# hzdr/PARIS

Hardware: AMD Instinct MI355X
Metric: GVoxel-updates/s (voxels x projections / s), FDK hot path weight+filter+backproject (higher is better)
Workload: dtype f32

## Files before the change

paris_amd/csrc/backproject.hip:

```cpp
#include "bp_device.h"

#include <mutex>
#include <utility>

namespace
{
    __global__ void __launch_bounds__(256) fastdiv_validate_kernel(float c, float r, unsigned long long* mismatches)
    {
        const uint32_t t = blockIdx.x * 256u + threadIdx.x;
        unsigned int bad = 0;
        for(uint32_t i = 0; i < 256u; ++i)
        {
            const uint32_t bits = (i << 24) | t;
            const float x = __uint_as_float(bits);
            const float want = x / c - (1.f / 2.f);
            const float got = div_by_constant(x, c, r) - (1.f / 2.f);
            const bool same = __float_as_uint(want) == __float_as_uint(got);
            const bool both_nan = (want != want) && (got != got);
            const bool want_far = !(fabsf(want) <= 16777216.f);
            const bool got_far = !(fabsf(got) <= 16777216.f);
            if(!(same || both_nan || (want_far && got_far)))
                ++bad;
        }
        if(bad)
// ... 256 lines not shown
}

int paris_hip_prevalidate_fast_division(paris_hip_ctx* ctx, float l_px_row, float l_px_col)
{
    if(ctx == nullptr || ctx->bp_fastdiv == 0)
        return PARIS_HIP_SUCCESS;
    bool ok = false;
    if(int rc = fastdiv_is_exact(ctx, l_px_row, &ok))
        return rc;
    return fastdiv_is_exact(ctx, l_px_col, &ok);
}

int paris_hip_prevalidate_lean_division(paris_hip_ctx* ctx, float d_so, float d_od)
{
    if(ctx == nullptr || ctx->bp_lean_div == 0)
        return PARIS_HIP_SUCCESS;
    bool ok = false;
    return paris_hip_lean_division_check(ctx, std::fabs(d_so) + std::fabs(d_od), d_so, &ok);
}

static int volume_stream_policy(const paris_hip_ctx* ctx, uint32_t v_dim_x, uint32_t v_dim_y, uint32_t v_dim_z)
{
    if(ctx->bp_nt >= 0)
        return ctx->bp_nt;
    const uint64_t bytes = 4ull * v_dim_x * v_dim_y * v_dim_z;
    return bytes <= (384ull << 20) ? 0 : 2;
}

static int fill_params(paris_hip_ctx* ctx, const void* d_p, bool f16, size_t p_pitch, uint32_t p_dim_x, uint32_t p_dim_y,
                       float* d_v, uint32_t v_dim_x, uint32_t v_dim_y, uint32_t v_dim_z, uint32_t v_offset,
                       const paris_detector_geometry* det_geo, const paris_volume_geometry* vol_geo, int enable_roi,
                       const paris_region_of_interest* roi, float sin_phi, float cos_phi, float delta_s, float delta_t,
                       BpParams& g, bool& fd, bool& skip)
{
    const size_t px = f16 ? sizeof(uint16_t) : sizeof(float);
    skip = false;
    if(int rc = paris_hip_bind(ctx))
        return rc;
    if(int rc = paris_hip_flush_pending_weight(ctx))
        return rc;
    if(d_p == nullptr || d_v == nullptr || det_geo == nullptr || vol_geo == nullptr || (enable_roi && roi == nullptr))
        return PARIS_HIP_ERROR_INVALID_ARGUMENT;
    if(p_dim_x == 0 || p_dim_y == 0 || p_pitch < static_cast<size_t>(p_dim_x) * px || p_pitch % px != 0)
        return PARIS_HIP_ERROR_INVALID_ARGUMENT;
    if(v_dim_x == 0 || v_dim_y == 0 || v_dim_z == 0)
    {
        skip = true;
        return PARIS_HIP_SUCCESS;
    }
    const uint64_t plane = static_cast<uint64_t>(v_dim_x) * v_dim_y;
    const uint32_t tz_auto = plane > (1ull << 20) ? (v_dim_z <= 256u ? 8u : TZ_DEFAULT) : (plane > (1ull << 18) ? 8u : TZ_DEFAULT);
    const uint32_t tz = ctx->bp_tz ? ctx->bp_tz : tz_auto;
    {
        const uint32_t tz_min = std::min(tz, 8u);
        const uint64_t ntx = (v_dim_x + 63u) / 64u, nty = (v_dim_y + 3u) / 4u, ntz = (v_dim_z + tz_min - 1u) / tz_min;
        const uint64_t zchunk = chunk_tiles(12u, tz_min, static_cast<uint32_t>(ntz), 64u);
        const uint64_t padded = std::max<uint64_t>(8ull * (8u * ((nty + 63u) / 64u)) * ntx * zchunk * ((ntz + zchunk - 1u) / zchunk),
                                                   8ull * ntx * nty * (ntz / 8u) + 8ull * 7u * 8u * ((nty + 63u) / 64u) * ntx);
        if(padded > 0x7fffff00ull)
            return PARIS_HIP_ERROR_UNSUPPORTED;
    }

    g = BpParams{};
    g.proj = d_p;
    g.proj_f16 = f16 ? 1u : 0u;
    g.vol = d_v;
    g.p_pitch = static_cast<uint32_t>(p_pitch / px);
    g.p_dim_x = p_dim_x;
    g.p_dim_y = p_dim_y;
    g.v_dim_x = v_dim_x;
    g.v_dim_y = v_dim_y;
    g.v_dim_z = v_dim_z;
    g.k_off = enable_roi ? roi->x1 : 0u;
    g.l_off = enable_roi ? roi->y1 : 0u;
    g.m_off = (enable_roi ? roi->z1 : 0u) + v_offset;
    g.x_base = centered_base(vol_geo->dim_x, vol_geo->l_vx_x);
    g.y_base = centered_base(vol_geo->dim_y, vol_geo->l_vx_y);
    g.z_base = centered_base(vol_geo->dim_z, vol_geo->l_vx_z);
    g.l_vx_x = vol_geo->l_vx_x;
    g.l_vx_y = vol_geo->l_vx_y;
    g.l_vx_z = vol_geo->l_vx_z;
    g.sin_phi = sin_phi;
    g.cos_phi = cos_phi;
    g.d_so = det_geo->d_so;
    g.d_sd = std::fabs(det_geo->d_so) + std::fabs(det_geo->d_od);
    g.l_px_x = det_geo->l_px_row;
    g.l_px_y = det_geo->l_px_col;
    g.min_h = detector_min(p_dim_x, g.l_px_x, delta_s);
    g.min_v = detector_min(p_dim_y, g.l_px_y, delta_t);
    g.rcp_l_px_y = 1.f / g.l_px_y;
    g.rcp_l_px_x = 1.f / g.l_px_x;
    fd = false;
    if(ctx->bp_fastdiv != 0)
    {
        bool fd_x = false;
        if(int rc = fastdiv_is_exact(ctx, g.l_px_y, &fd))
            return rc;
        if(int rc = fastdiv_is_exact(ctx, g.l_px_x, &fd_x))
            return rc;
        fd = fd && fd_x;
    }
    {
        const double x0 = g.x_base + static_cast<double>(g.k_off) * g.l_vx_x, x1 = g.x_base + (static_cast<double>(g.k_off) + v_dim_x - 1.0) * g.l_vx_x;
        const double y0 = g.y_base + static_cast<double>(g.l_off) * g.l_vx_y, y1 = g.y_base + (static_cast<double>(g.l_off) + v_dim_y - 1.0) * g.l_vx_y;
        const double reach = std::hypot(std::max(std::fabs(x0), std::fabs(x1)), std::max(std::fabs(y0), std::fabs(y1)));
        const double lo = std::ldexp(1.0, -40), hi = std::ldexp(1.0, 40);
        const bool ordinary = g.d_so >= lo && g.d_so <= hi && g.d_sd >= lo && g.d_sd <= hi;
        g.lean_div = (ctx->bp_lean_div != 0 && ordinary && std::isfinite(reach) && reach <= 0.9 * g.d_so) ? 1u : 0u;
        if(g.lean_div != 0u)
        {
            bool exact = false;
            if(int rc = paris_hip_lean_division_check(ctx, g.d_sd, g.d_so, &exact))
// ... 10 lines not shown
    {
#ifdef PARIS_HIP_EXPERIMENTS
        static const int tile_nest = std::getenv("PARIS_TILE_NEST") ? std::atoi(std::getenv("PARIS_TILE_NEST")) : -1;
#else
        constexpr int tile_nest = -1;
#endif
        g.yfast = tile_nest >= 0 ? static_cast<uint32_t>(tile_nest) : (v_dim_z > 256u ? 2u : 0u);
    }
    g.order = ctx->bp_order >= 0 ? static_cast<uint32_t>(ctx->bp_order) : (plane > (1ull << 20) ? 15u : 18u);
    g.store_sc1 = volume_stream_policy(ctx, v_dim_x, v_dim_y, v_dim_z) == 2 ? 1u : 0u;
    g.stage_vec4 = (ctx->bp_stage_vec4 != 0 && g.p_pitch % 4u == 0 && reinterpret_cast<uintptr_t>(d_p) % (4u * px) == 0)
                       ? 1u : 0u;
    return PARIS_HIP_SUCCESS;
}

static int lane_width(const float* d_v, uint32_t v_dim_x)
{
    const uintptr_t addr = reinterpret_cast<uintptr_t>(d_v);
    if(v_dim_x % 4u == 0 && addr % 16u == 0)
        return 4;
    if(v_dim_x % 2u == 0 && addr % 8u == 0)
        return 2;
    return 1;
}

static int backproject_impl(paris_hip_ctx* ctx, const void* d_p, bool f16, size_t p_pitch, uint32_t p_dim_x,
                            uint32_t p_dim_y, float* d_v, uint32_t v_dim_x, uint32_t v_dim_y, uint32_t v_dim_z,
                            uint32_t v_offset, const paris_detector_geometry* det_geo,
                            const paris_volume_geometry* vol_geo, int enable_roi, const paris_region_of_interest* roi,
                            float sin_phi, float cos_phi, float delta_s, float delta_t)
{
    BpParams g;
    bool fd = false, skip = false;
    if(int rc = fill_params(ctx, d_p, f16, p_pitch, p_dim_x, p_dim_y, d_v, v_dim_x, v_dim_y, v_dim_z, v_offset, det_geo, vol_geo,
                            enable_roi, roi, sin_phi, cos_phi, delta_s, delta_t, g, fd, skip))
        return rc;
    if(skip)
        return paris_hip_finish(ctx);

    const bool timed = !ctx->bp_start.empty();
    const size_t ev = timed ? static_cast<size_t>(ctx->bp_launches % ctx->bp_start.size()) : 0u;
    if(timed)
        PARIS_HIP_TRY(hipEventRecord(ctx->bp_start[ev], ctx->stream));
    if(ctx->bp_variant == 4 && !f16)
    {
        FusedParams fp{};
        fp.g = g;
        fp.n_proj = 1;
        fp.proj_tab[0] = d_p;
        fp.sin_phi[0] = sin_phi;
        fp.cos_phi[0] = cos_phi;
        const int width = lane_width(d_v, v_dim_x);
        const int vx = ctx->bp_vx == 4 && width == 4 ? 4 : (ctx->bp_vx == 1 || width < 2 ? 1 : 2);
        paris_hip_bp_launch_fused(&fp, vx, ctx->bp_tz == 8u ? 8 : (ctx->bp_tz == 32u ? 32 : 16), volume_stream_policy(ctx, v_dim_x, v_dim_y, v_dim_z) != 0, fd, ctx->stream);
    }
    else
    if(ctx->bp_variant == 1)
    {
        const dim3 grid((v_dim_x + 255u) / 256u, v_dim_y, v_dim_z);
        if(v_dim_y > 65535u || v_dim_z > 65535u)
            return PARIS_HIP_ERROR_UNSUPPORTED;
        hipLaunchKernelGGL(bp_gather_kernel, grid, dim3(256), 0, ctx->stream, g);
    }
    else
    {
        int vx = lane_width(d_v, v_dim_x);
        if(ctx->bp_vx && ctx->bp_vx < vx)
            vx = ctx->bp_vx;
        if(ctx->bp_vx == 0 && vx == 4 && ctx->bp_variant != 3 && ctx->bp_variant != 5)
        {
            const uint64_t tiles = static_cast<uint64_t>((v_dim_x + 63u) / 64u) * ((v_dim_y + 15u) / 16u) * ((v_dim_z + g.tz - 1u) / g.tz);
            if(tiles < 2048u)
                vx = 2;
        }
        const bool deep_big = g.tz == 16u && ctx->bp_tz == 0u && static_cast<uint64_t>(v_dim_x) * v_dim_y > (1ull << 20);
        if(deep_big && ctx->bp_unroll == 0 && ctx->bp_lds_bytes == 0u && vx == 4)
            g.lds_floats = 40u * 1024u / sizeof(float);
        const int unroll = ctx->bp_unroll ? ctx->bp_unroll : ((g.tz == 8u && ctx->bp_tz == 0u) || (deep_big && ctx->bp_lds_bytes == 0u && vx == 4) ? 1 : 2);
        const bool nt = volume_stream_policy(ctx, v_dim_x, v_dim_y, v_dim_z) != 0;
#ifdef PARIS_HIP_EXPERIMENTS
        const bool want_slice = ctx->bp_variant == 3;
        if(want_slice && vx == 4)
        {
            const int nw = ctx->bp_slice_nw ? ctx->bp_slice_nw : 16;
            const int rpl = ctx->bp_slice_rpl ? ctx->bp_slice_rpl : 4;
            const uint32_t box_bytes = ctx->bp_lds_bytes ? ctx->bp_lds_bytes : LDS_BYTES_DEFAULT;
            if(int rc = launch_slice_shape(g, nw, rpl, box_bytes, nt, fd, ctx->stream))
                return rc;
        }
        else if(vx == 4 && ctx->bp_variant == 5 && v_dim_y <= 65535u)
        {
            const size_t need = 3u * static_cast<size_t>(v_dim_x) * v_dim_y;
            if(ctx->colstate_floats < need)
            {
                if(ctx->colstate != nullptr)
                {
                    PARIS_HIP_TRY(hipStreamSynchronize(ctx->stream));
                    PARIS_HIP_TRY(hipFree(ctx->colstate));
                    ctx->colstate = nullptr;
                }
                PARIS_HIP_TRY(hipMalloc(reinterpret_cast<void**>(&ctx->colstate), need * sizeof(float)));
                ctx->colstate_floats = need;
            }
            g.colstate = ctx->colstate;
            if(unroll == 1)
                fd ? launch_tile_pre<1, true>(g, ctx->stream) : launch_tile_pre<1, false>(g, ctx->stream);
            else
// ... 491 lines not shown
    hipLaunchKernelGGL(to_half_kernel, grid, dim3(256), 0, ctx->stream, d_src, static_cast<uint32_t>(src_pitch / sizeof(float)),
                       reinterpret_cast<_Float16*>(d_dst), static_cast<uint32_t>(dst_pitch / sizeof(uint16_t)), dim_x, dim_y);
    if(int rc = paris_hip_note_projection_use(ctx, d_src, src_pitch * dim_y))
        return rc;
    if(int rc = paris_hip_note_projection_use(ctx, d_dst, dst_pitch * dim_y))
        return rc;
    return paris_hip_finish(ctx);
}

extern "C" int paris_hip_backproject_batch(paris_hip_ctx* ctx, const float* d_p, size_t p_pitch,
                                           size_t p_stride_bytes, uint32_t n_proj, uint32_t p_dim_x,
                                           uint32_t p_dim_y, float* d_v, uint32_t v_dim_x, uint32_t v_dim_y,
                                           uint32_t v_dim_z, uint32_t v_offset,
                                           const paris_detector_geometry* det_geo,
                                           const paris_volume_geometry* vol_geo, int enable_roi,
                                           const paris_region_of_interest* roi, const float* sin_phi,
                                           const float* cos_phi, float delta_s, float delta_t)
{
    if(int rc = paris_hip_flush_deferred(ctx))
        return rc;
    return batch_impl(ctx, d_p, false, p_pitch, p_stride_bytes, n_proj, p_dim_x, p_dim_y, d_v, v_dim_x, v_dim_y, v_dim_z, v_offset, det_geo,
                      vol_geo, enable_roi, roi, sin_phi, cos_phi, delta_s, delta_t);
}

extern "C" int paris_hip_backproject_batch_f16(paris_hip_ctx* ctx, const uint16_t* d_p, size_t p_pitch, size_t p_stride_bytes,
                                               uint32_t n_proj, uint32_t p_dim_x, uint32_t p_dim_y, float* d_v, uint32_t v_dim_x,
                                               uint32_t v_dim_y, uint32_t v_dim_z, uint32_t v_offset,
                                               const paris_detector_geometry* det_geo, const paris_volume_geometry* vol_geo,
                                               int enable_roi, const paris_region_of_interest* roi, const float* sin_phi,
                                               const float* cos_phi, float delta_s, float delta_t)
{
    if(int rc = paris_hip_flush_deferred(ctx))
        return rc;
    return batch_impl(ctx, d_p, true, p_pitch, p_stride_bytes, n_proj, p_dim_x, p_dim_y, d_v, v_dim_x, v_dim_y, v_dim_z, v_offset, det_geo,
                      vol_geo, enable_roi, roi, sin_phi, cos_phi, delta_s, delta_t);
}

static int batch_impl(paris_hip_ctx* ctx, const void* d_p, bool f16, size_t p_pitch, size_t p_stride_bytes, uint32_t n_proj, uint32_t p_dim_x,
                      uint32_t p_dim_y, float* d_v, uint32_t v_dim_x, uint32_t v_dim_y, uint32_t v_dim_z, uint32_t v_offset,
                      const paris_detector_geometry* det_geo, const paris_volume_geometry* vol_geo, int enable_roi,
                      const paris_region_of_interest* roi, const float* sin_phi, const float* cos_phi, float delta_s, float delta_t,
                      const void* const* ptrs)
{
    const size_t px = f16 ? sizeof(uint16_t) : sizeof(float);
    if(ctx == nullptr || sin_phi == nullptr || cos_phi == nullptr || (ptrs == nullptr && p_stride_bytes % px != 0))
        return PARIS_HIP_ERROR_INVALID_ARGUMENT;
    if(n_proj == 0)
        return paris_hip_finish(ctx);
    if(ptrs == nullptr && n_proj > 1 && p_stride_bytes < p_pitch * static_cast<size_t>(p_dim_y))
        return PARIS_HIP_ERROR_INVALID_ARGUMENT;
    const auto where = [&](uint32_t i) { return ptrs != nullptr ? static_cast<const char*>(ptrs[i]) : static_cast<const char*>(d_p) + static_cast<size_t>(i) * p_stride_bytes; };

    const int width = d_v != nullptr ? lane_width(d_v, v_dim_x) : 1;
    bool deep_box_fits = true;
    {
        const double d_so = std::fabs(static_cast<double>(det_geo->d_so)), d_sd = d_so + std::fabs(static_cast<double>(det_geo->d_od));
        const double mag = d_so > 0.0 ? d_sd / d_so : 1.0;
        const double rows = 32.0 * vol_geo->l_vx_z * mag / det_geo->l_px_col + 4.0 * std::max(vol_geo->l_vx_x, vol_geo->l_vx_y) * mag / det_geo->l_px_col + 8.0;
        const double cols = 64.0 * std::max(vol_geo->l_vx_x, vol_geo->l_vx_y) * mag / det_geo->l_px_row + 16.0;
        const double budget = ctx->bp_lds_bytes != 0u ? ctx->bp_lds_bytes : 32.0 * 1024.0;
        deep_box_fits = std::isfinite(rows) && std::isfinite(cols) && rows * std::max(132.0, cols) * sizeof(float) <= budget;
    }
    int fused_vx = ((v_dim_z <= 16u || !deep_box_fits) && width >= 2) ? 2 : 1;
    if(ctx->bp_vx == 4 && width == 4)
        fused_vx = 4;
    else if(ctx->bp_vx == 2 && width >= 2)
        fused_vx = 2;
    else if(ctx->bp_vx == 1)
        fused_vx = 1;
    int fused_tz = fused_vx == 1 ? ((v_dim_z <= 16u || !deep_box_fits) ? 16 : 32) : 16;
    if(ctx->bp_tz == 8u && fused_vx != 1)
        fused_tz = 8;
    else if(ctx->bp_tz == 16u)
        fused_tz = 16;
    else if(ctx->bp_tz == 32u && fused_vx == 1)
        fused_tz = 32;
    const bool fused_ok = n_proj > 1 && (ctx->bp_variant == 0 || ctx->bp_variant == 4) && d_v != nullptr;
    if(!fused_ok)
    {
        const unsigned saved = ctx->flags;
        ctx->flags &= ~PARIS_HIP_CTX_SYNCHRONOUS;
        int rc = PARIS_HIP_SUCCESS;
        for(uint32_t i = 0; i < n_proj && rc == PARIS_HIP_SUCCESS; ++i)
        {
            const char* p = where(i);
            rc = backproject_impl(ctx, p, f16, p_pitch, p_dim_x, p_dim_y, d_v, v_dim_x, v_dim_y, v_dim_z, v_offset, det_geo, vol_geo,
                                  enable_roi, roi, sin_phi[i], cos_phi[i], delta_s, delta_t);
        }
        ctx->flags = saved;
        if(rc != PARIS_HIP_SUCCESS)
            return rc;
        return paris_hip_finish(ctx);
    }

    const bool nt = volume_stream_policy(ctx, v_dim_x, v_dim_y, v_dim_z) != 0;
    for(uint32_t first = 0; first < n_proj; first += FUSED_MAX)
    {
        const uint32_t n = std::min<uint32_t>(FUSED_MAX, n_proj - first);
        FusedParams fp{};
        bool fd = false, skip = false;
        const char* p0 = where(first);
        if(int rc = fill_params(ctx, p0, f16, p_pitch, p_dim_x, p_dim_y, d_v, v_dim_x, v_dim_y, v_dim_z, v_offset, det_geo,
                                vol_geo, enable_roi, roi, sin_phi[first], cos_phi[first], delta_s, delta_t, fp.g, fd, skip))
            return rc;
        if(skip)
            break;
        fp.n_proj = n;
        if(ctx->bp_order < 0 && fp.g.order == 15u)
            fp.g.order = fused_vx == 1 ? 17u : (fused_vx == 2 ? 16u : 15u);
#ifdef PARIS_HIP_EXPERIMENTS
        static const bool x_fast = std::getenv("PARIS_FUSED_XFAST") != nullptr;
#else
        constexpr bool x_fast = false;
#endif
        fp.g.yfast = x_fast ? 0u : 1u;
        if(ctx->bp_lds_bytes == 0u)
            fp.g.lds_floats = 32u * 1024u / sizeof(float);
        for(uint32_t i = 0; i < n; ++i)
        {
            fp.sin_phi[i] = sin_phi[first + i];
            fp.cos_phi[i] = cos_phi[first + i];
            fp.proj_tab[i] = where(first + i);
            if(reinterpret_cast<uintptr_t>(fp.proj_tab[i]) % (4u * px) != 0)
                fp.g.stage_vec4 = 0u;
        }
        for(uint32_t i = n; i < FUSED_MAX; ++i)
            fp.proj_tab[i] = fp.proj_tab[0];
        const bool timed = !ctx->bp_start.empty();
        const size_t ev = timed ? static_cast<size_t>(ctx->bp_launches % ctx->bp_start.size()) : 0u;
        if(timed)
            PARIS_HIP_TRY(hipEventRecord(ctx->bp_start[ev], ctx->stream));
        paris_hip_bp_launch_fused(&fp, fused_vx, fused_tz, nt, fd, ctx->stream);
        if(timed)
            PARIS_HIP_TRY(hipEventRecord(ctx->bp_stop[ev], ctx->stream));
        ++ctx->bp_launches;
        for(uint32_t i = 0; i < n && !ctx->upload_targets.empty(); ++i)
            if(int rc = paris_hip_note_projection_use(ctx, where(first + i), p_pitch * p_dim_y))
                return rc;
    }
    return paris_hip_finish(ctx);
}

extern "C" int paris_hip_last_backproject_ms(paris_hip_ctx* ctx, float* ms)
{
    if(int rc = paris_hip_flush_deferred(ctx))
        return rc;
    if(ctx == nullptr || ms == nullptr || ctx->bp_launches == 0 || ctx->bp_start.empty())
        return PARIS_HIP_ERROR_INVALID_ARGUMENT;
    if(int rc = paris_hip_bind(ctx))
        return rc;
    const size_t ev = static_cast<size_t>((ctx->bp_launches - 1) % ctx->bp_start.size());
    PARIS_HIP_TRY(hipEventSynchronize(ctx->bp_stop[ev]));
    PARIS_HIP_TRY(hipEventElapsedTime(ms, ctx->bp_start[ev], ctx->bp_stop[ev]));
    return PARIS_HIP_SUCCESS;
}

extern "C" int paris_hip_set_backproject_variant(paris_hip_ctx* ctx, int variant)
{
    if(int rc = paris_hip_flush_deferred(ctx))
        return rc;
    if(ctx == nullptr || variant < 0 || variant > 5)
        return PARIS_HIP_ERROR_INVALID_ARGUMENT;
#ifndef PARIS_HIP_EXPERIMENTS
    if(variant == 3 || variant == 5)
        return PARIS_HIP_ERROR_UNSUPPORTED;
#endif
    ctx->bp_variant = variant;
    return PARIS_HIP_SUCCESS;
}

extern "C" int paris_hip_set_backproject_order(paris_hip_ctx* ctx, int order, int nontemporal)
{
    if(int rc = paris_hip_flush_deferred(ctx))
        return rc;
    if(ctx == nullptr || !(order == -1 || order == 0 || order == 1 || order == 5 || order == 8 || order == 9 || order == 12 || (order >= 14 && order <= 18)) || nontemporal < -1 || nontemporal > 2)
        return PARIS_HIP_ERROR_INVALID_ARGUMENT;
#ifndef PARIS_HIP_EXPERIMENTS
    if(order == 0 || order == 1 || order == 8 || order == 9 || order == 12)
        return PARIS_HIP_ERROR_UNSUPPORTED;
#endif
    ctx->bp_order = order;
    ctx->bp_nt = nontemporal;
    return PARIS_HIP_SUCCESS;
}

// ... 1 lines not shown
{
    if(int rc = paris_hip_bind(ctx))
        return rc;
    if(exact == nullptr)
        return PARIS_HIP_ERROR_INVALID_ARGUMENT;
    bool ok = false;
    const int saved = ctx->async_validate;
    ctx->async_validate = 0;
    const int rc = fastdiv_is_exact(ctx, divisor, &ok);
    ctx->async_validate = saved;
    if(rc != PARIS_HIP_SUCCESS)
        return rc;
    *exact = ok ? 1 : 0;
    return PARIS_HIP_SUCCESS;
}

extern "C" int paris_hip_set_backproject_vector_staging(paris_hip_ctx* ctx, int enable)
{
    if(int rc = paris_hip_flush_deferred(ctx))
        return rc;
    if(ctx == nullptr)
        return PARIS_HIP_ERROR_INVALID_ARGUMENT;
    ctx->bp_stage_vec4 = enable ? 1 : 0;
    return PARIS_HIP_SUCCESS;
}

extern "C" int paris_hip_set_backproject_skip_invalid(paris_hip_ctx* ctx, int enable)
{
    if(int rc = paris_hip_flush_deferred(ctx))
        return rc;
    if(ctx == nullptr)
        return PARIS_HIP_ERROR_INVALID_ARGUMENT;
    ctx->bp_skip_invalid = enable ? 1 : 0;
    return PARIS_HIP_SUCCESS;
}

extern "C" int paris_hip_set_backproject_fast_division(paris_hip_ctx* ctx, int enable)
{
    if(int rc = paris_hip_flush_deferred(ctx))
        return rc;
    if(ctx == nullptr)
        return PARIS_HIP_ERROR_INVALID_ARGUMENT;
    ctx->bp_lean_div = enable ? 1 : 0;
    ctx->bp_fastdiv = enable ? 1 : 0;
    return PARIS_HIP_SUCCESS;
}

extern "C" int paris_hip_set_backproject_slice_shape(paris_hip_ctx* ctx, int waves, int row_groups)
{
    if(int rc = paris_hip_flush_deferred(ctx))
        return rc;
    if(ctx == nullptr)
        return PARIS_HIP_ERROR_INVALID_ARGUMENT;
    const bool ok = (waves == 0 && row_groups == 0) || (waves == 16 && (row_groups == 4 || row_groups == 2))
                    || (waves == 8 && (row_groups == 4 || row_groups == 2 || row_groups == 1));
    if(!ok)
        return PARIS_HIP_ERROR_INVALID_ARGUMENT;
#ifndef PARIS_HIP_EXPERIMENTS
    if(waves != 0)
        return PARIS_HIP_ERROR_UNSUPPORTED;
#endif
    ctx->bp_slice_nw = waves;
    ctx->bp_slice_rpl = row_groups;
    return PARIS_HIP_SUCCESS;
}

extern "C" int paris_hip_set_backproject_tuning(paris_hip_ctx* ctx, int vx, int unroll, int tz, int lds_bytes)
{
    if(int rc = paris_hip_flush_deferred(ctx))
        return rc;
    if(ctx == nullptr)
        return PARIS_HIP_ERROR_INVALID_ARGUMENT;
    if(!(vx == 0 || vx == 1 || vx == 2 || vx == 4) || !(unroll == 0 || unroll == 1 || unroll == 2 || unroll == 3 || unroll == 4))
        return PARIS_HIP_ERROR_INVALID_ARGUMENT;
    if(tz < 0 || tz > 4096 || lds_bytes < 0 || lds_bytes > static_cast<int>(LDS_BYTES_MAX)
       || (lds_bytes != 0 && lds_bytes < 1024))
        return PARIS_HIP_ERROR_INVALID_ARGUMENT;
#ifndef PARIS_HIP_EXPERIMENTS
    if(unroll > 2)
        return PARIS_HIP_ERROR_UNSUPPORTED;
#endif
    ctx->bp_vx = vx;
    ctx->bp_unroll = unroll;
    ctx->bp_tz = static_cast<uint32_t>(tz);
    ctx->bp_lds_bytes = static_cast<uint32_t>(lds_bytes);
    return PARIS_HIP_SUCCESS;
}

extern "C" int paris_hip_has_experiments(void)
{
#ifdef PARIS_HIP_EXPERIMENTS
    return 1;
#else
    return 0;
#endif
}
```

paris_amd/csrc/backproject_fused.hip:

```cpp
#define PARIS_BP_SINGLE_INSTRUCTION_FLOOR 1
#if (defined(PARIS_TIMING_ONLY_NO_BARRIERS) || defined(PARIS_TIMING_ONLY_STAGE_ONCE)) && !defined(PARIS_HIP_EXPERIMENTS)
#error "the timing-only switches compute WRONG results: they exist in the experiments build only (make EXPERIMENTS=1)"
#endif
#include "bp_device.h"

namespace
{
#ifndef PARIS_FUSED_PIPELINE
#define PARIS_FUSED_PIPELINE 1
#endif
#ifndef PARIS_FUSED_WAVES
#define PARIS_FUSED_WAVES 3
#endif
    constexpr int FIXED_STRIDE = 132;

    template <int VX, int TZ, bool NT, bool FD>
    __global__ void __launch_bounds__(256, PARIS_FUSED_WAVES + (VX == 2 ? 1 : VX == 1 ? (TZ == 32 ? 1 : 4) : 0) + (TZ == 8 ? 1 : 0)) bp_fused_kernel(const FusedParams fp)
    {
        extern __shared__ __attribute__((aligned(16))) float lds[];
        BpParams g = fp.g;
        using vec = typename vec_of<VX>::type;
        constexpr uint32_t XL = 64u / VX;
        constexpr uint32_t RW = VX;
        constexpr uint32_t TY = 4u * RW;

        const uint32_t tid = threadIdx.x;
        const uint32_t lane = tid & 63u;
        const uint32_t wave = tid >> 6;

        uint32_t bx, by, bz;
        if(!tile_of_block(g, blockIdx.x, bx, by, bz))
            return;
        const uint32_t k0 = bx * 64u;
        const uint32_t l0 = by * TY;
        const uint32_t m0 = bz * TZ;
        const uint32_t k1 = min(k0 + 63u, g.v_dim_x - 1u);
        const uint32_t l1 = min(l0 + TY - 1u, g.v_dim_y - 1u);
        const uint32_t m1 = min(m0 + TZ - 1u, g.v_dim_z - 1u);
        const uint32_t mcount = m1 - m0 + 1u;

        const uint32_t xq = lane % XL, yy = lane / XL;
        const uint32_t k = k0 + xq * VX;
        const uint32_t l = l0 + wave * RW + yy;
        const bool active = k < g.v_dim_x && l < g.v_dim_y;

        const size_t slice = static_cast<size_t>(g.v_dim_x) * g.v_dim_y;
        float* vp = g.vol + (static_cast<size_t>(m0) * g.v_dim_y + l) * g.v_dim_x + k;
        vec acc[TZ] = {};
#pragma unroll
        for(int z = 0; z < TZ; ++z)
            if(active && static_cast<uint32_t>(z) < mcount)
                acc[z] = load_voxels<VX, NT>(vp + z * slice);

        const float z_first = g.z_base + static_cast<float>(g.m_off + m0) * g.l_vx_z;
        const float z_last = g.z_base + static_cast<float>(g.m_off + m1) * g.l_vx_z;
        __shared__ int box_tab[FUSED_MAX * BOX_WORDS];
        if(wave * 16u < fp.n_proj)
            tile_boxes_to_lds(g, fp.sin_phi, fp.cos_phi, wave * 16u, fp.n_proj, k0, k1, l0, l1, m0, m1, lane, g.lds_floats, FIXED_STRIDE, box_tab);
        for(uint32_t p = 0; p < fp.n_proj; ++p)
        {
            g.sin_phi = fp.sin_phi[p];
            g.cos_phi = fp.cos_phi[p];
            g.proj = fp.proj_tab[p];
#ifdef PARIS_TIMING_ONLY_NO_BARRIERS
            if(p == 0u)
#endif
            __syncthreads();
            const Box box = box_from_lds(box_tab, p, lane);
#ifdef PARIS_TIMING_ONLY_STAGE_ONCE
            if(p == 0u)
#endif
            stage_box(g, box, lds, wave, 4u, lane);
#ifdef PARIS_TIMING_ONLY_NO_BARRIERS
            if(p == 0u)
#endif
            __syncthreads();
            {
                Column col[VX];
                bool all_fast = true, all_inside = true, all_none = true;
#pragma unroll
                for(int j = 0; j < VX; ++j)
                {
                    col[j] = make_column<FD>(g, box, g.k_off + min(k + j, k1), g.l_off + min(l, l1), z_first, z_last);
                    all_fast = all_fast && col[j].fast;
                    all_inside = all_inside && col[j].inside;
                    all_none = all_none && col[j].none;
                }
                auto add_projection = [&](auto fast_tag, auto full_tag, auto inside_tag, auto stride_tag) {
                    constexpr bool FAST = decltype(fast_tag)::value;
                    constexpr bool FULL = decltype(full_tag)::value;
                    constexpr bool INSIDE = decltype(inside_tag)::value;
                    constexpr int CS = decltype(stride_tag)::value;
                    if constexpr(FAST && FULL && PARIS_FUSED_PIPELINE > 0)
                    {
                        constexpr int AHEAD = PARIS_FUSED_PIPELINE;
                        Tap ring[AHEAD + 1][VX];
                        auto fetch = [&](int z) {
                            const float z_m = g.z_base + static_cast<float>(g.m_off + m0 + static_cast<uint32_t>(z)) * g.l_vx_z;
#pragma unroll
                            for(int j = 0; j < VX; ++j)
                                ring[z % (AHEAD + 1)][j] = fetch_tap<FD, INSIDE, CS>(g, box, lds, z_m, col[j]);
                        };
#pragma unroll
                        for(int z = 0; z < AHEAD && z < TZ; ++z)
                            fetch(z);
#pragma unroll
                        for(int z = 0; z < TZ; ++z)
                        {
                            if(z + AHEAD < TZ)
                                fetch(z + AHEAD);
#pragma unroll
                            for(int j = 0; j < VX; ++j)
                                elem<VX>(acc[z], j) += finish_tap<INSIDE>(col[j], ring[z % (AHEAD + 1)][j]);
                        }
                        return;
                    }
#pragma unroll
                    for(int z = 0; z < TZ; ++z)
                    {
                        if(FULL || static_cast<uint32_t>(z) < mcount)
                        {
                            const float z_m = g.z_base + static_cast<float>(g.m_off + m0 + z) * g.l_vx_z;
#pragma unroll
                            for(int j = 0; j < VX; ++j)
                                elem<VX>(acc[z], j) += voxel_contribution<FD, FAST, INSIDE, CS>(g, box, lds, z_m, col[j]);
                        }
                    }
                };
                const bool wave_inside = mcount == TZ && g.p_dim_y < (1u << 23) && __all(all_inside ? 1 : 0) != 0;
                const bool fixed = box.stride == FIXED_STRIDE;
                using no_stride = std::integral_constant<int, 0>;
                using the_stride = std::integral_constant<int, FIXED_STRIDE>;
                if(g.skip_invalid != 0u && __all(all_none ? 1 : 0) != 0)
                {
                }
                else if(wave_inside && fixed)
                    add_projection(std::true_type{}, std::true_type{}, std::true_type{}, the_stride{});
                else if(wave_inside)
                    add_projection(std::true_type{}, std::true_type{}, std::true_type{}, no_stride{});
                else if(all_fast && mcount == TZ && fixed)
                    add_projection(std::true_type{}, std::true_type{}, std::false_type{}, the_stride{});
                else if(all_fast && mcount == TZ)
                    add_projection(std::true_type{}, std::true_type{}, std::false_type{}, no_stride{});
                else if(all_fast)
                    add_projection(std::true_type{}, std::false_type{}, std::false_type{}, no_stride{});
                else
                    add_projection(std::false_type{}, std::false_type{}, std::false_type{}, no_stride{});
            }
        }
#pragma unroll
        for(int z = 0; z < TZ; ++z)
            if(active && static_cast<uint32_t>(z) < mcount)
                store_voxels<VX, NT>(vp + z * slice, acc[z], g.store_sc1 != 0u);
    }

    template <int VX, int TZ, bool NT, bool FD>
    void launch_fused(FusedParams& fp, hipStream_t stream)
    {
        BpParams& g = fp.g;
        g.tz = TZ;
        g.ntx = (g.v_dim_x + 63u) / 64u;
        g.nty = (g.v_dim_y + 4u * VX - 1u) / (4u * VX);
        g.ntz = (g.v_dim_z + TZ - 1u) / TZ;
        settle_order(g);
        g.zchunk = chunk_tiles(g.order, TZ, g.ntz, 32u);
        const uint32_t blocks = static_cast<uint32_t>(grid_blocks(g));
        hipLaunchKernelGGL((bp_fused_kernel<VX, TZ, NT, FD>), dim3(blocks), dim3(256), g.lds_floats * sizeof(float), stream, fp);
    }

    template <int VX, int TZ>
    void launch_fused_flags(FusedParams& fp, bool nt, bool fd, hipStream_t stream)
    {
        if(nt && fd)
            launch_fused<VX, TZ, true, true>(fp, stream);
        else if(nt)
            launch_fused<VX, TZ, true, false>(fp, stream);
        else if(fd)
            launch_fused<VX, TZ, false, true>(fp, stream);
        else
            launch_fused<VX, TZ, false, false>(fp, stream);
    }
}

void paris_hip_bp_launch_fused(const void* fused_params, int vx, int tz, bool nt, bool fd, hipStream_t stream)
{
    FusedParams fp = *static_cast<const FusedParams*>(fused_params);
    if(vx == 1 && tz == 32)
        launch_fused_flags<1, 32>(fp, nt, fd, stream);
    else if(vx == 1)
        launch_fused_flags<1, 16>(fp, nt, fd, stream);
    else if(vx == 2 && tz == 8)
        launch_fused_flags<2, 8>(fp, nt, fd, stream);
    else if(vx == 2)
        launch_fused_flags<2, 16>(fp, nt, fd, stream);
    else if(tz == 8)
        launch_fused_flags<4, 8>(fp, nt, fd, stream);
    else
        launch_fused_flags<4, 16>(fp, nt, fd, stream);
}

void paris_hip_warm_backproject_fused()
{
    hipFuncAttributes a{};
    (void)hipFuncGetAttributes(&a, reinterpret_cast<const void*>((&bp_fused_kernel<1, 32, true, true>)));
}
```

paris_amd/csrc/bp_device.h:

```cpp
#ifndef PARIS_HIP_BP_DEVICE_H_
#define PARIS_HIP_BP_DEVICE_H_

#include "paris_hip_internal.h"
#include "ieee_lean.h"

#include <algorithm>
#include <cmath>
#include <cstdlib>
#include <cstring>
#include <type_traits>

#ifndef PARIS_BP_SINGLE_INSTRUCTION_FLOOR
#define PARIS_BP_SINGLE_INSTRUCTION_FLOOR 0
#endif

namespace
{
    struct BpParams
    {
        const void* proj;
        uint32_t proj_f16;
        float* vol;
        uint32_t p_pitch;
        uint32_t p_dim_x, p_dim_y;
// ... 44 lines not shown
        ColConst c;
        float so_over_den;
        if(g.lean_div)
        {
            const float r = paris_lean::refined_rcp(den);
            c.factor = paris_lean::div_with_rcp(g.d_sd, den, r);
            so_over_den = paris_lean::div_with_rcp(g.d_so, den, r);
        }
        else
        {
            c.factor = g.d_sd / den;
            so_over_den = g.d_so / den;
        }
        const float b = (t * c.factor) - g.min_h;
        const float q = FD ? div_by_constant(b, g.l_px_x, g.rcp_l_px_x) : b / g.l_px_x;
        c.h = q - (1.f / 2.f);
        c.u = -so_over_den;
        return c;
    }

    template <bool FD>
    __device__ __forceinline__ float v_coordinate(const BpParams& g, float z_m, float factor)
    {
        const float b = (z_m * factor) - g.min_v;
        const float q = FD ? div_by_constant(b, g.l_px_y, g.rcp_l_px_y) : b / g.l_px_y;
        return q - (1.f / 2.f);
    }

    __device__ __forceinline__ int to_int_clamped(float x)
    {
        x = fminf(fmaxf(x, -1.0e9f), 1.0e9f);
        return static_cast<int>(floorf(x));
    }

    template <int VX> struct vec_of;
    template <> struct vec_of<1> { using type = float; };
    template <> struct vec_of<2> { using type = float2; };
    template <> struct vec_of<4> { using type = float4; };

    template <int VX> __device__ __forceinline__ float& elem(typename vec_of<VX>::type& v, int j);
    template <> __device__ __forceinline__ float& elem<1>(float& v, int) { return v; }
    template <> __device__ __forceinline__ float& elem<2>(float2& v, int j) { return j == 0 ? v.x : v.y; }
    template <> __device__ __forceinline__ float& elem<4>(float4& v, int j)
    {
        return j == 0 ? v.x : (j == 1 ? v.y : (j == 2 ? v.z : v.w));
    }

    __host__ __device__ inline uint32_t dealt_band(uint32_t nty, uint32_t order)
    {
        const uint32_t grp = 1u << (order - 14u);
        return grp * ((nty + 8u * grp - 1u) / (8u * grp));
    }

    __host__ __device__ inline uint32_t order18_tail_group_log2(const BpParams& g)
    {
        return g.yfast == 1u ? 3u : 1u;
    }

    inline uint64_t grid_blocks(const BpParams& g)
    {
        const uint64_t total = static_cast<uint64_t>(g.ntx) * g.nty * g.ntz;
        if(g.order == 5u)
            return ((total + 7u) / 8u) * 8u;
#ifdef PARIS_HIP_EXPERIMENTS
        if(g.order == 8u || g.order == 9u)
            return 8ull * ((g.nty + 7u) / 8u) * g.ntx * g.ntz;
        if(g.order == 12u)
            return 8ull * ((g.nty + 7u) / 8u) * g.ntx * g.zchunk * ((g.ntz + g.zchunk - 1u) / g.zchunk);
#endif
        if(g.order == 18u)
            return 8ull * (static_cast<uint64_t>(g.ntx) * g.nty * (g.ntz / 8u)
                           + static_cast<uint64_t>(g.ntz % 8u) * dealt_band(g.nty, 14u + order18_tail_group_log2(g)) * g.ntx);
        if(g.order >= 14u && g.order <= 17u)
            return 8ull * dealt_band(g.nty, g.order) * g.ntx * g.zchunk * ((g.ntz + g.zchunk - 1u) / g.zchunk);
        return total;
    }

    inline void settle_order(BpParams& g)
    {
        if(g.order == 18u && g.ntz < 8u)
            g.order = 5u;
    }

    inline uint32_t chunk_tiles(uint32_t order, uint32_t tz, uint32_t ntz, uint32_t deep)
    {
        const uint32_t slices = order >= 14u ? deep : 256u;
        return std::min(std::max(1u, slices / std::max(1u, tz)), std::max(1u, ntz));
    }

    template <int VX> struct ext_of;
    template <> struct ext_of<1> { typedef float type; };
    template <> struct ext_of<2> { typedef float type __attribute__((ext_vector_type(2))); };
    template <> struct ext_of<4> { typedef float type __attribute__((ext_vector_type(4))); };

    template <int VX, bool NT> __device__ __forceinline__ typename vec_of<VX>::type load_voxels(const float* p)
    {
        using ext_t = typename ext_of<VX>::type;
        using vec_t = typename vec_of<VX>::type;
        ext_t e = NT ? __builtin_nontemporal_load(reinterpret_cast<const ext_t*>(p)) : *reinterpret_cast<const ext_t*>(p);
        return *reinterpret_cast<vec_t*>(&e);
    }
    template <int VX, bool NT> __device__ __forceinline__ void store_voxels(float* p, typename vec_of<VX>::type v, bool sc1 = true)
    {
        using ext_t = typename ext_of<VX>::type;
        const ext_t e = *reinterpret_cast<ext_t*>(&v);
        if(NT && VX == 4 && sc1)
        {
            asm volatile("global_store_dwordx4 %0, %1, off sc1 nt\n\ts_nop 1" ::"v"(p), "v"(e) : "memory");
        }
        else if(NT)
            __builtin_nontemporal_store(e, reinterpret_cast<ext_t*>(p));
        else
            *reinterpret_cast<ext_t*>(p) = e;
    }

    __device__ __forceinline__ bool tile_of_block(const BpParams& g, uint32_t b, uint32_t& bx, uint32_t& by, uint32_t& bz)
    {
        const uint32_t total = g.ntx * g.nty * g.ntz;
#ifdef PARIS_HIP_EXPERIMENTS
        if(g.order == 1u)
        {
            if(b >= total)
                return false;
            bz = b % g.ntz;
            b /= g.ntz;
            bx = b % g.ntx;
            by = b / g.ntx;
            return true;
        }
        if(g.order == 8u)
        {
            const uint32_t band = (g.nty + 7u) / 8u;
            const uint32_t xcd = b % 8u;
            uint32_t r = b / 8u;
            bx = r % g.ntx;
            r /= g.ntx;
            bz = r % g.ntz;
            const uint32_t yb = r / g.ntz;
            by = xcd * band + yb;
            return yb < band && by < g.nty;
        }
#endif
        if(g.order == 18u)
        {
            const uint32_t xcd = b % 8u;
            uint32_t r = b / 8u;
            const uint32_t full = g.ntz / 8u, plane = g.ntx * g.nty;
            if(r >= full * plane)
            {
                r -= full * plane;
                const uint32_t lg = order18_tail_group_log2(g), grp = 1u << lg;
                const uint32_t band = dealt_band(g.nty, 14u + lg);
                uint32_t yb;
                if(g.yfast == 1u)
                {
                    const uint32_t yl = r % grp;
                    r /= grp;
                    bx = r % g.ntx;
                    r /= g.ntx;
                    const uint32_t ngrp = band / grp;
                    yb = (r % ngrp) * grp + yl;
                    r /= ngrp;
                }
                else
                {
                    bx = r % g.ntx;
                    r /= g.ntx;
                    yb = r % band;
                    r /= band;
                }
                bz = full * 8u + r;
                by = (yb / grp) * (8u * grp) + xcd * grp + yb % grp;
                return bz < g.ntz && by < g.nty;
            }
            if(g.yfast == 1u)
            {
                by = r % g.nty;
                r /= g.nty;
                bx = r % g.ntx;
                bz = (r / g.ntx) * 8u + xcd;
            }
            else
            {
                bx = r % g.ntx;
                r /= g.ntx;
                by = r % g.nty;
                bz = (r / g.nty) * 8u + xcd;
            }
            return bz < g.ntz;
        }
        if(g.order >= 14u && g.order <= 17u)
        {
            const uint32_t band = dealt_band(g.nty, g.order);
            const uint32_t grp = 1u << (g.order - 14u);
            const uint32_t zchunk = g.zchunk;
            const uint32_t xcd = b % 8u;
            uint32_t r = b / 8u;
            uint32_t zl, yb;
            if(g.yfast == 2u)
            {
                bx = r % g.ntx;
                r /= g.ntx;
                const uint32_t yl = r % grp;
                r /= grp;
// ... 474 lines not shown
        using lds_cptr = const __attribute__((address_space(3))) float*;
        const int stride4 = (CS != 0 ? CS : b.stride) << 2;
        const uint32_t xaddr = static_cast<uint32_t>(reinterpret_cast<uintptr_t>(lds_box)) + (static_cast<uint32_t>(max(col.xoff, 0)) << 2);
        uint32_t a1;
        if(ALLVALID)
        {
            t.valid = true;
            uint32_t xrel = xaddr - static_cast<uint32_t>(__mul24(b.by0, stride4));
            asm("" : "+v"(xrel));
            a1 = static_cast<uint32_t>(__mul24(y1i, stride4)) + xrel;
        }
        else
        {
            const int rrel = y1i - b.by0;
            const unsigned rowlim = col.ymax > 0.f ? static_cast<unsigned>(max(b.bhs - 1, 0)) : 0u;
            t.valid = static_cast<unsigned>(rrel) < rowlim;
            int rc;
            asm("v_med3_i32 %0, %1, 0, %2" : "=v"(rc) : "v"(rrel), "v"(max(b.bhs - 2, 0)));
            a1 = static_cast<uint32_t>(__mul24(rc, stride4)) + xaddr;
        }
        lds_cptr r1 = reinterpret_cast<lds_cptr>(a1);
        lds_cptr r2 = CS != 0 ? r1 + CS : reinterpret_cast<lds_cptr>(a1 + static_cast<uint32_t>(stride4));
        t.q11 = r1[0];
        t.q21 = r1[1];
        t.q12 = r2[0];
        t.q22 = r2[1];
        return t;
    }

    template <bool ALLVALID>
    __device__ __forceinline__ float finish_tap(const Column& col, const Tap& t)
    {
        const float interp_y1 = col.wx2 * t.q11 + col.wx1 * t.q21;
        const float interp_y2 = col.wx2 * t.q12 + col.wx1 * t.q22;
        const float wy2 = 1.f - t.wy1;
        float det = wy2 * interp_y1 + t.wy1 * interp_y2;
        if(!ALLVALID)
            det = t.valid ? det : 0.f;
        return 0.5f * det * col.u * col.u;
    }

    constexpr int FUSED_MAX = 64;

    struct FusedParams
    {
        BpParams g;
        uint32_t n_proj;
        float sin_phi[FUSED_MAX];
        float cos_phi[FUSED_MAX];
        const void* proj_tab[FUSED_MAX];
    };
}

void paris_hip_bp_launch_fused(const void* fused_params, int vx, int tz, bool nt, bool fd, hipStream_t stream);

#endif
```

paris_amd/csrc/paris_hip_internal.h:

```cpp
#ifndef PARIS_HIP_INTERNAL_H_
#define PARIS_HIP_INTERNAL_H_

#include <hip/hip_runtime.h>

#include <cstddef>
#include <array>
#include <cstdint>
#include <map>
#include <vector>

#include "paris_hip.h"

#pragma clang fp contract(off)

#define PARIS_HIP_TRY(expr)                                   \
    do                                                        \
    {                                                         \
        hipError_t paris_hip_err__ = (expr);                  \
        if(paris_hip_err__ != hipSuccess)                     \
            return static_cast<int>(paris_hip_err__);         \
    } while(0)

struct paris_hip_fft_plan
{
    float2* d_twiddle = nullptr;
    float2* d_tab_first = nullptr;
    float2* d_tab_mid[3] = {nullptr, nullptr, nullptr};
};

struct paris_hip_filter_info
{
    uint32_t size = 0;
    float* d_kp = nullptr;
};

struct paris_hip_ctx
{
    int device = 0;
    hipStream_t stream = nullptr;
    bool owns_stream = false;
    unsigned flags = 0;
    std::vector<hipEvent_t> bp_start, bp_stop;
    uint64_t bp_launches = 0;
    int bp_variant = 0;
    int bp_vx = 0, bp_unroll = 0;
    uint32_t bp_tz = 0, bp_lds_bytes = 0;
    int bp_order = -1;
    int bp_slice_nw = 0, bp_slice_rpl = 0;
    int bp_nt = -1;
    int bp_stage_vec4 = 1;
    int bp_fastdiv = 1;
    int bp_skip_invalid = 1;
    std::map<uintptr_t, size_t> clean_volumes;
    std::map<uintptr_t, size_t> volume_allocs;
    int bp_lean_div = 1;
    std::map<uint32_t, bool> fastdiv_exact;
    std::map<std::array<uint32_t, 4>, bool> lean_checks;
    int lean_validate = 1;
    bool filter_lds_attr_set = false;
    bool filter_r16_attr_set[5] = {false, false, false, false, false};
    int filter_variant = 0;
    std::map<uint32_t, paris_hip_fft_plan> plans;
    std::map<const float*, paris_hip_filter_info> filters;
    int stage_fusion = 0;
    struct pending_weight_t
    {
        bool active = false;
        float* d_p = nullptr;
        size_t pitch = 0;
        uint32_t dim_x = 0, dim_y = 0, row_first = 0, row_count = 0;
        float h_min = 0.f, v_min = 0.f, d_sd = 0.f, l_px_row = 0.f, l_px_col = 0.f;
        bool filter = false;
        const float* d_kp = nullptr;
        const paris_hip_fft_plan* plan = nullptr;
        uint32_t filter_size = 0;
    } pending_weight;
    int filter_deferral = 0;
    std::vector<pending_weight_t> defer_wf;
    hipStream_t upload_stream = nullptr;
    std::vector<hipEvent_t> upload_events;
    uint64_t uploads = 0;
    struct upload_target
    {
        hipEvent_t last_use = nullptr;
        bool used = false;
        size_t bytes = 0;
    };
    std::map<const void*, upload_target> upload_targets;
    struct flat_field_t
    {
        float* d_ref = nullptr;
        uint32_t dim_x = 0, dim_y = 0;
        double t_min = 1.0;
        std::vector<uint8_t> dead;
    } flat_field;
    struct defect_map_t
    {
        bool set = false;
        uint32_t* d_plan = nullptr;
        uint32_t dim_x = 0, dim_y = 0;
        uint32_t n = 0, m = 0;
// ... 225 lines not shown
```

Measured before the change: 785.6.

## Add square 16x16 voxel footprint for fused backprojection kernel

Adds a template parameter for the fused backprojection kernel so a tile can be 16 columns by 16 rows instead of 64 by 4. It uses a narrower LDS detector box stride. The square footprint is chosen automatically when vx=1, tz=32 and a geometry estimate says the LDS detector box fits, or it can be forced through a config knob. The aim is a smaller projected detector footprint per tile, which means less LDS staging and better reuse of cached projection data. In exchange there are narrower x-rows per wave, which may hurt coalescing of volume stores. The block ordering also changes to order 15.

```diff
diff --git a/paris_amd/csrc/backproject.hip b/paris_amd/csrc/backproject.hip
--- a/paris_amd/csrc/backproject.hip
+++ b/paris_amd/csrc/backproject.hip
@@ -332,12 +332,13 @@
     const uint32_t tz_auto = plane > (1ull << 20) ? (v_dim_z <= 256u ? 8u : TZ_DEFAULT) : (plane > (1ull << 18) ? 8u : TZ_DEFAULT);
     const uint32_t tz = ctx->bp_tz ? ctx->bp_tz : tz_auto;
     {
-        const uint32_t tz_min = std::min(tz, 8u);
-        const uint64_t ntx = (v_dim_x + 63u) / 64u, nty = (v_dim_y + 3u) / 4u, ntz = (v_dim_z + tz_min - 1u) / tz_min;
-        const uint64_t zchunk = chunk_tiles(12u, tz_min, static_cast<uint32_t>(ntz), 64u);
-        const uint64_t padded = std::max<uint64_t>(8ull * (8u * ((nty + 63u) / 64u)) * ntx * zchunk * ((ntz + zchunk - 1u) / zchunk),
-                                                   8ull * ntx * nty * (ntz / 8u) + 8ull * 7u * 8u * ((nty + 63u) / 64u) * ntx);
-        if(padded > 0x7fffff00ull)
+        const auto padded = [&](uint32_t tw, uint32_t ty, uint32_t tz_min) {
+            const uint64_t ntx = (v_dim_x + tw - 1u) / tw, nty = (v_dim_y + ty - 1u) / ty, ntz = (v_dim_z + tz_min - 1u) / tz_min;
+            const uint64_t zchunk = chunk_tiles(12u, tz_min, static_cast<uint32_t>(ntz), 64u);
+            return std::max<uint64_t>(8ull * (8u * ((nty + 63u) / 64u)) * ntx * zchunk * ((ntz + zchunk - 1u) / zchunk),
+                                      8ull * ntx * nty * (ntz / 8u) + 8ull * 7u * 8u * ((nty + 63u) / 64u) * ntx);
+        };
+        if(std::max(padded(64u, 4u, std::min(tz, 8u)), padded(16u, 16u, 32u)) > 0x7fffff00ull)
             return PARIS_HIP_ERROR_UNSUPPORTED;
     }
 
@@ -454,7 +455,7 @@
         fp.cos_phi[0] = cos_phi;
         const int width = lane_width(d_v, v_dim_x);
         const int vx = ctx->bp_vx == 4 && width == 4 ? 4 : (ctx->bp_vx == 1 || width < 2 ? 1 : 2);
-        paris_hip_bp_launch_fused(&fp, vx, ctx->bp_tz == 8u ? 8 : (ctx->bp_tz == 32u ? 32 : 16), volume_stream_policy(ctx, v_dim_x, v_dim_y, v_dim_z) != 0, fd, ctx->stream);
+        paris_hip_bp_launch_fused(&fp, vx, ctx->bp_tz == 8u ? 8 : (ctx->bp_tz == 32u ? 32 : 16), ctx->bp_fused_rows == 16 ? 16 : 64, volume_stream_policy(ctx, v_dim_x, v_dim_y, v_dim_z) != 0, fd, ctx->stream);
     }
     else
     if(ctx->bp_variant == 1)
@@ -1052,7 +1053,7 @@
     const auto where = [&](uint32_t i) { return ptrs != nullptr ? static_cast<const char*>(ptrs[i]) : static_cast<const char*>(d_p) + static_cast<size_t>(i) * p_stride_bytes; };
 
     const int width = d_v != nullptr ? lane_width(d_v, v_dim_x) : 1;
-    bool deep_box_fits = true;
+    bool deep_box_fits = true, square_box_fits = true;
     {
         const double d_so = std::fabs(static_cast<double>(det_geo->d_so)), d_sd = d_so + std::fabs(static_cast<double>(det_geo->d_od));
         const double mag = d_so > 0.0 ? d_sd / d_so : 1.0;
@@ -1060,6 +1061,9 @@
         const double cols = 64.0 * std::max(vol_geo->l_vx_x, vol_geo->l_vx_y) * mag / det_geo->l_px_row + 16.0;
         const double budget = ctx->bp_lds_bytes != 0u ? ctx->bp_lds_bytes : 32.0 * 1024.0;
         deep_box_fits = std::isfinite(rows) && std::isfinite(cols) && rows * std::max(132.0, cols) * sizeof(float) <= budget;
+        const double rows_sq = rows + 12.0 * std::max(vol_geo->l_vx_x, vol_geo->l_vx_y) * mag / det_geo->l_px_col;
+        const double cols_sq = 16.0 * std::sqrt(2.0) * std::max(vol_geo->l_vx_x, vol_geo->l_vx_y) * mag / det_geo->l_px_row + 16.0;
+        square_box_fits = std::isfinite(rows_sq) && std::isfinite(cols_sq) && rows_sq * std::max(68.0, cols_sq) * sizeof(float) <= budget;
     }
     int fused_vx = ((v_dim_z <= 16u || !deep_box_fits) && width >= 2) ? 2 : 1;
     if(ctx->bp_vx == 4 && width == 4)
@@ -1075,6 +1079,12 @@
         fused_tz = 16;
     else if(ctx->bp_tz == 32u && fused_vx == 1)
         fused_tz = 32;
+    if(ctx->bp_fused_rows == 16)
+    {
+        fused_vx = 1;
+        fused_tz = 32;
+    }
+    const int fused_tw = (fused_vx == 1 && fused_tz == 32 && (ctx->bp_fused_rows == 16 || (ctx->bp_fused_rows == 0 && square_box_fits))) ? 16 : 64;
     const bool fused_ok = n_proj > 1 && (ctx->bp_variant == 0 || ctx->bp_variant == 4) && d_v != nullptr;
     if(!fused_ok)
     {
@@ -1107,7 +1117,7 @@
             break;
         fp.n_proj = n;
         if(ctx->bp_order < 0 && fp.g.order == 15u)
-            fp.g.order = fused_vx == 1 ? 17u : (fused_vx == 2 ? 16u : 15u);
+            fp.g.order = fused_tw == 16 ? 15u : (fused_vx == 1 ? 17u : (fused_vx == 2 ? 16u : 15u));
 #ifdef PARIS_HIP_EXPERIMENTS
         static const bool x_fast = std::getenv("PARIS_FUSED_XFAST") != nullptr;
 #else
@@ -1130,7 +1140,7 @@
         const size_t ev = timed ? static_cast<size_t>(ctx->bp_launches % ctx->bp_start.size()) : 0u;
         if(timed)
             PARIS_HIP_TRY(hipEventRecord(ctx->bp_start[ev], ctx->stream));
-        paris_hip_bp_launch_fused(&fp, fused_vx, fused_tz, nt, fd, ctx->stream);
+        paris_hip_bp_launch_fused(&fp, fused_vx, fused_tz, fused_tw, nt, fd, ctx->stream);
         if(timed)
             PARIS_HIP_TRY(hipEventRecord(ctx->bp_stop[ev], ctx->stream));
         ++ctx->bp_launches;
@@ -1238,10 +1248,17 @@
         return rc;
     if(ctx == nullptr)
         return PARIS_HIP_ERROR_INVALID_ARGUMENT;
+    const bool fused_footprint = waves == 4 && (row_groups == 16 || row_groups == 4);
     const bool ok = (waves == 0 && row_groups == 0) || (waves == 16 && (row_groups == 4 || row_groups == 2))
-                    || (waves == 8 && (row_groups == 4 || row_groups == 2 || row_groups == 1));
+                    || (waves == 8 && (row_groups == 4 || row_groups == 2 || row_groups == 1)) || fused_footprint;
     if(!ok)
         return PARIS_HIP_ERROR_INVALID_ARGUMENT;
+    if(fused_footprint)
+    {
+        ctx->bp_fused_rows = row_groups;
+        return PARIS_HIP_SUCCESS;
+    }
+    ctx->bp_fused_rows = 0;
 #ifndef PARIS_HIP_EXPERIMENTS
     if(waves != 0)
         return PARIS_HIP_ERROR_UNSUPPORTED;
diff --git a/paris_amd/csrc/backproject_fused.hip b/paris_amd/csrc/backproject_fused.hip
--- a/paris_amd/csrc/backproject_fused.hip
+++ b/paris_amd/csrc/backproject_fused.hip
@@ -13,28 +13,31 @@
 #define PARIS_FUSED_WAVES 3
 #endif
     constexpr int FIXED_STRIDE = 132;
-
-    template <int VX, int TZ, bool NT, bool FD>
+    constexpr int NARROW_STRIDE = 68;
+
+    template <int VX, int TZ, int XL, bool NT, bool FD>
     __global__ void __launch_bounds__(256, PARIS_FUSED_WAVES + (VX == 2 ? 1 : VX == 1 ? (TZ == 32 ? 1 : 4) : 0) + (TZ == 8 ? 1 : 0)) bp_fused_kernel(const FusedParams fp)
     {
         extern __shared__ __attribute__((aligned(16))) float lds[];
         BpParams g = fp.g;
         using vec = typename vec_of<VX>::type;
-        constexpr uint32_t XL = 64u / VX;
-        constexpr uint32_t RW = VX;
+        static_assert(XL * VX == 64 || (XL == 16 && VX == 1), "footprints: 64 columns wide, or 16 x 16");
+        constexpr uint32_t TW = XL * VX;
+        constexpr uint32_t RW = 64u / XL;
         constexpr uint32_t TY = 4u * RW;
+        constexpr int STRIDE = TW == 64u ? FIXED_STRIDE : NARROW_STRIDE;
 
         const uint32_t tid = threadIdx.x;
         const uint32_t lane = tid & 63u;
         const uint32_t wave = tid >> 6;
 
         uint32_t bx, by, bz;
-        if(!tile_of_block(g, blockIdx.x, bx, by, bz))
+        if(!tile_of_block(g, blockIdx.x, bx, by, bz, TW))
             return;
-        const uint32_t k0 = bx * 64u;
+        const uint32_t k0 = bx * TW;
         const uint32_t l0 = by * TY;
         const uint32_t m0 = bz * TZ;
-        const uint32_t k1 = min(k0 + 63u, g.v_dim_x - 1u);
+        const uint32_t k1 = min(k0 + TW - 1u, g.v_dim_x - 1u);
         const uint32_t l1 = min(l0 + TY - 1u, g.v_dim_y - 1u);
         const uint32_t m1 = min(m0 + TZ - 1u, g.v_dim_z - 1u);
         const uint32_t mcount = m1 - m0 + 1u;
@@ -56,7 +59,7 @@
         const float z_last = g.z_base + static_cast<float>(g.m_off + m1) * g.l_vx_z;
         __shared__ int box_tab[FUSED_MAX * BOX_WORDS];
         if(wave * 16u < fp.n_proj)
-            tile_boxes_to_lds(g, fp.sin_phi, fp.cos_phi, wave * 16u, fp.n_proj, k0, k1, l0, l1, m0, m1, lane, g.lds_floats, FIXED_STRIDE, box_tab);
+            tile_boxes_to_lds(g, fp.sin_phi, fp.cos_phi, wave * 16u, fp.n_proj, k0, k1, l0, l1, m0, m1, lane, g.lds_floats, STRIDE, box_tab);
         for(uint32_t p = 0; p < fp.n_proj; ++p)
         {
             g.sin_phi = fp.sin_phi[p];
@@ -128,9 +131,9 @@
                     }
                 };
                 const bool wave_inside = mcount == TZ && g.p_dim_y < (1u << 23) && __all(all_inside ? 1 : 0) != 0;
-                const bool fixed = box.stride == FIXED_STRIDE;
+                const bool fixed = box.stride == STRIDE;
                 using no_stride = std::integral_constant<int, 0>;
-                using the_stride = std::integral_constant<int, FIXED_STRIDE>;
+                using the_stride = std::integral_constant<int, STRIDE>;
                 if(g.skip_invalid != 0u && __all(all_none ? 1 : 0) != 0)
                 {
                 }
@@ -154,38 +157,41 @@
                 store_voxels<VX, NT>(vp + z * slice, acc[z], g.store_sc1 != 0u);
     }
 
-    template <int VX, int TZ, bool NT, bool FD>
+    template <int VX, int TZ, int XL, bool NT, bool FD>
     void launch_fused(FusedParams& fp, hipStream_t stream)
     {
+        constexpr uint32_t TW = XL * VX, TY = 4u * (64u / XL);
         BpParams& g = fp.g;
         g.tz = TZ;
-        g.ntx = (g.v_dim_x + 63u) / 64u;
-        g.nty = (g.v_dim_y + 4u * VX - 1u) / (4u * VX);
+        g.ntx = (g.v_dim_x + TW - 1u) / TW;
+        g.nty = (g.v_dim_y + TY - 1u) / TY;
         g.ntz = (g.v_dim_z + TZ - 1u) / TZ;
         settle_order(g);
         g.zchunk = chunk_tiles(g.order, TZ, g.ntz, 32u);
-        const uint32_t blocks = static_cast<uint32_t>(grid_blocks(g));
-        hipLaunchKernelGGL((bp_fused_kernel<VX, TZ, NT, FD>), dim3(blocks), dim3(256), g.lds_floats * sizeof(float), stream, fp);
+        const uint32_t blocks = static_cast<uint32_t>(grid_blocks(g, TW));
+        hipLaunchKernelGGL((bp_fused_kernel<VX, TZ, XL, NT, FD>), dim3(blocks), dim3(256), g.lds_floats * sizeof(float), stream, fp);
     }
 
-    template <int VX, int TZ>
+    template <int VX, int TZ, int XL = 64 / VX>
     void launch_fused_flags(FusedParams& fp, bool nt, bool fd, hipStream_t stream)
     {
         if(nt && fd)
-            launch_fused<VX, TZ, true, true>(fp, stream);
+            launch_fused<VX, TZ, XL, true, true>(fp, stream);
         else if(nt)
-            launch_fused<VX, TZ, true, false>(fp, stream);
+            launch_fused<VX, TZ, XL, true, false>(fp, stream);
         else if(fd)
-            launch_fused<VX, TZ, false, true>(fp, stream);
+            launch_fused<VX, TZ, XL, false, true>(fp, stream);
         else
-            launch_fused<VX, TZ, false, false>(fp, stream);
+            launch_fused<VX, TZ, XL, false, false>(fp, stream);
     }
 }
 
-void paris_hip_bp_launch_fused(const void* fused_params, int vx, int tz, bool nt, bool fd, hipStream_t stream)
+void paris_hip_bp_launch_fused(const void* fused_params, int vx, int tz, int tile_width, bool nt, bool fd, hipStream_t stream)
 {
     FusedParams fp = *static_cast<const FusedParams*>(fused_params);
-    if(vx == 1 && tz == 32)
+    if(vx == 1 && tz == 32 && tile_width == 16)
+        launch_fused_flags<1, 32, 16>(fp, nt, fd, stream);
+    else if(vx == 1 && tz == 32)
         launch_fused_flags<1, 32>(fp, nt, fd, stream);
     else if(vx == 1)
         launch_fused_flags<1, 16>(fp, nt, fd, stream);
@@ -202,5 +208,5 @@
 void paris_hip_warm_backproject_fused()
 {
     hipFuncAttributes a{};
-    (void)hipFuncGetAttributes(&a, reinterpret_cast<const void*>((&bp_fused_kernel<1, 32, true, true>)));
+    (void)hipFuncGetAttributes(&a, reinterpret_cast<const void*>((&bp_fused_kernel<1, 32, 64, true, true>)));
 }
diff --git a/paris_amd/csrc/bp_device.h b/paris_amd/csrc/bp_device.h
--- a/paris_amd/csrc/bp_device.h
+++ b/paris_amd/csrc/bp_device.h
@@ -120,12 +120,12 @@
         return grp * ((nty + 8u * grp - 1u) / (8u * grp));
     }
 
-    __host__ __device__ inline uint32_t order18_tail_group_log2(const BpParams& g)
-    {
-        return g.yfast == 1u ? 3u : 1u;
-    }
-
-    inline uint64_t grid_blocks(const BpParams& g)
+    __host__ __device__ inline uint32_t order18_tail_group_log2(const BpParams& g, uint32_t tw = 64u)
+    {
+        return (g.yfast == 1u && tw != 16u) ? 3u : 1u;
+    }
+
+    inline uint64_t grid_blocks(const BpParams& g, uint32_t tw = 64u)
     {
         const uint64_t total = static_cast<uint64_t>(g.ntx) * g.nty * g.ntz;
         if(g.order == 5u)
@@ -138,7 +138,7 @@
 #endif
         if(g.order == 18u)
             return 8ull * (static_cast<uint64_t>(g.ntx) * g.nty * (g.ntz / 8u)
-                           + static_cast<uint64_t>(g.ntz % 8u) * dealt_band(g.nty, 14u + order18_tail_group_log2(g)) * g.ntx);
+                           + static_cast<uint64_t>(g.ntz % 8u) * dealt_band(g.nty, 14u + order18_tail_group_log2(g, tw)) * g.ntx);
         if(g.order >= 14u && g.order <= 17u)
             return 8ull * dealt_band(g.nty, g.order) * g.ntx * g.zchunk * ((g.ntz + g.zchunk - 1u) / g.zchunk);
         return total;
@@ -182,7 +182,7 @@
             *reinterpret_cast<ext_t*>(p) = e;
     }
 
-    __device__ __forceinline__ bool tile_of_block(const BpParams& g, uint32_t b, uint32_t& bx, uint32_t& by, uint32_t& bz)
+    __device__ __forceinline__ bool tile_of_block(const BpParams& g, uint32_t b, uint32_t& bx, uint32_t& by, uint32_t& bz, uint32_t tw = 64u)
     {
         const uint32_t total = g.ntx * g.nty * g.ntz;
 #ifdef PARIS_HIP_EXPERIMENTS
@@ -217,7 +217,7 @@
             if(r >= full * plane)
             {
                 r -= full * plane;
-                const uint32_t lg = order18_tail_group_log2(g), grp = 1u << lg;
+                const uint32_t lg = order18_tail_group_log2(g, tw), grp = 1u << lg;
                 const uint32_t band = dealt_band(g.nty, 14u + lg);
                 uint32_t yb;
                 if(g.yfast == 1u)
@@ -798,6 +798,6 @@
     };
 }
 
-void paris_hip_bp_launch_fused(const void* fused_params, int vx, int tz, bool nt, bool fd, hipStream_t stream);
+void paris_hip_bp_launch_fused(const void* fused_params, int vx, int tz, int tile_width, bool nt, bool fd, hipStream_t stream);
 
 #endif
diff --git a/paris_amd/csrc/paris_hip_internal.h b/paris_amd/csrc/paris_hip_internal.h
--- a/paris_amd/csrc/paris_hip_internal.h
+++ b/paris_amd/csrc/paris_hip_internal.h
@@ -47,6 +47,7 @@
     uint32_t bp_tz = 0, bp_lds_bytes = 0;
     int bp_order = -1;
     int bp_slice_nw = 0, bp_slice_rpl = 0;
+    int bp_fused_rows = 0;
     int bp_nt = -1;
     int bp_stage_vec4 = 1;
     int bp_fastdiv = 1;
```

Result: no change. 785.7 (median of 4 runs) (+0.0%).
